# tech-srl/code2vec

Hardware: NVIDIA H100
Metric: path-contexts/sec (train step, batch 1024x200) (higher is better)
Workload: dtype tf32 operands / fp32 accumulate+storage

## Files before the change

### code2vec_b200/csrc/engine.cu

```cuda
#include <cuda_runtime.h>
#include <math.h>
#include <stdio.h>
#include <stdlib.h>
#include <string.h>

#include <string>
#include <utility>
#include <vector>

#include "../../include/c2v_b200.h"
#include "common.cuh"
#include "kernels.cuh"
#include "sgemm.cuh"
#include "umma_gemm.cuh"

using namespace c2v;

namespace {

thread_local std::string g_create_error = "";

constexpr size_t kAlign = 256;
inline size_t align_up(size_t x, size_t a = kAlign) { return (x + a - 1) / a * a; }

constexpr int kSplitDv = 18;
constexpr int kSplitDw = 48;

struct Workspace {
  size_t H, Xg, dXg, alpha, v, dv, S, loss_b, lse, loss, part, da_part, lse_part, dl;
  size_t Xg_lo, H_lo, S_lo, tgt_hi, tgt_lo, W_hi, W_lo, v_hi, v_lo;
  size_t WT, WT_lo, vT, vT_lo, tgtT, tgtT_lo;
  size_t true_logit, rscale, v_scaled, slab_flag;
  size_t st_src, st_pth, st_tgt, st_mask, st_target, st_topk_idx, st_topk_val, st_code, st_attn;
  size_t nx_src, nx_pth, nx_tgt;
  size_t sb_src, sb_pth, sb_tgt, sb_mask, sb_target;
  size_t stamp_tok, stamp_path, last_tok, last_path, lr_tab;
  size_t stamp_tgt, last_tgt;
  size_t perm, bkt_count, bkt_cursor, bkt_starts;
  size_t det_keys[2], det_vals[2], det_hist, det_offs, det_starts, det_part;
  size_t total;
  size_t ldS;
  size_t ldB;
};

bool dims_ok(const c2v_dims* d, std::string* why) {
  auto bad = [&](const char* m) { if (why) *why = m; return false; };
  if (!d) return bad("dims is NULL");
  if (d->token_vocab < 1 || d->path_vocab < 1 || d->target_vocab < 1) return bad("vocab sizes must be >= 1");
  if (d->embed_dim < 4 || d->embed_dim % 4) return bad("embed_dim must be a positive multiple of 4");
  if (d->code_dim < 4 || d->code_dim % 4 || d->code_dim > 1024) return bad("code_dim must be a multiple of 4 in [4, 1024]");
  if (d->max_contexts < 1) return bad("max_contexts must be >= 1");
  if (d->max_batch < 1) return bad("max_batch must be >= 1");
  if (d->top_k < 1 || d->top_k > 64) return bad("top_k must be in [1, 64]");
  if ((double)d->max_batch * d->max_contexts > 2.0e9) return bad("max_batch * max_contexts overflows int32");
  return true;
}

Workspace carve(const c2v_dims& d) {
  Workspace w{};
  const size_t N = (size_t)d.max_batch * d.max_contexts, D = d.code_dim, B = d.max_batch, X = 3 * (size_t)d.embed_dim;
  w.ldS = align_up((size_t)d.target_vocab, 64);
  w.ldB = align_up(B, 4);
  size_t off = 0;
  auto take = [&](size_t bytes) { size_t o = off; off = align_up(off + bytes); return o; };
  w.H = take(N * D * 4);
  w.Xg = take(N * X * 4);
  w.dXg = take(N * X * 4);
  w.alpha = take(N * 4);
  w.v = take(B * D * 4);
  w.dv = take(B * D * 4);
  w.S = take(B * w.ldS * 4);
  w.loss_b = take(B * 4);
  w.lse = take(B * 4);
  w.true_logit = take(B * 4);
  w.rscale = take(B * 4);
  w.v_scaled = take(B * D * 4);
  w.slab_flag = take(64);
  w.loss = take(64);
  size_t part = (size_t)kSplitDv * B * D;
  if ((size_t)kSplitDw * X * D > part) part = (size_t)kSplitDw * X * D;
  w.part = take(part * 4);
  w.da_part = take(B * D * 4);
  w.lse_part = take(B * (size_t)umma::lse_slots(d.target_vocab) * 8);
  w.dl = take(B * (size_t)(kMaxSampled + 1) * 4);
  w.st_src = take(N * 4);
  w.st_pth = take(N * 4);
  w.st_tgt = take(N * 4);
  w.st_mask = take(N * 4);
  w.nx_src = take(N * 4);
  w.nx_pth = take(N * 4);
  w.nx_tgt = take(N * 4);
  w.st_target = take(B * 4);
  w.sb_src = take(N * 4);
  w.sb_pth = take(N * 4);
  w.sb_tgt = take(N * 4);
  w.sb_mask = take(N * 4);
  w.sb_target = take(B * 4);
  w.st_topk_idx = take(B * (size_t)d.top_k * 4);
  w.st_topk_val = take(B * (size_t)d.top_k * 4);
  w.st_code = take(B * D * 4);
  w.st_attn = take(N * 4);
  w.stamp_tok = take((size_t)d.token_vocab * 4);
  w.stamp_path = take((size_t)d.path_vocab * 4);
  w.last_tok = take((size_t)d.token_vocab * 4);
  w.last_path = take((size_t)d.path_vocab * 4);
  w.lr_tab = take((size_t)kLrRing * 4);
  w.perm = take(3 * N * 4);
  w.bkt_count = take((size_t)kMaxBuckets * 4);
  w.bkt_cursor = take((size_t)kMaxBuckets * 4);
  w.bkt_starts = take((size_t)(kMaxBuckets + 1) * 4);
  w.stamp_tgt = take((size_t)d.target_vocab * 4);
  w.last_tgt = take((size_t)d.target_vocab * 4);
  w.Xg_lo = take(N * X * 4);
  w.H_lo = take(N * D * 4);
  w.S_lo = take(B * w.ldS * 4);
  w.tgt_hi = take((size_t)d.target_vocab * D * 4);
  w.tgt_lo = take((size_t)d.target_vocab * D * 4);
  w.W_hi = take(X * D * 4);
  w.W_lo = take(X * D * 4);
  w.v_hi = take(B * D * 4);
  w.v_lo = take(B * D * 4);
  w.WT = take(X * D * 4);
  w.WT_lo = take(X * D * 4);
  w.vT = take(D * w.ldB * 4);
  w.vT_lo = take(D * w.ldB * 4);
  w.tgtT = take(D * w.ldS * 4);
  w.tgtT_lo = take(D * w.ldS * 4);
  const size_t M = 3 * N, tiles = (M + kDetSortTile - 1) / kDetSortTile;
  for (int i = 0; i < 2; ++i) { w.det_keys[i] = take(M * 4); w.det_vals[i] = take(M * 4); }
  w.det_hist = take(kDetRadix * tiles * 4);
  w.det_offs = take(kDetRadix * tiles * 4);
  w.det_starts = take((kDetRadix * tiles + 1) * 4);
  w.det_part = take(2 * ((M + kDetChunk - 1) / kDetChunk) * (size_t)d.embed_dim * 4);
  w.total = off;
  return w;
}

}

enum Phase { PH_CTX_FWD = 0, PH_ATTN_FWD, PH_LOGITS, PH_XENT, PH_DV, PH_DY, PH_ATTN_BWD, PH_DW, PH_DX_SCATTER,
             PH_ADAM, PH_TOPK, PH_SAMPLED, PH_GATHER, PH_DX_GEMM, PH_ADAM_CATCHUP, PH_SPLIT, PH_ADAM_SWEEP, PH_PEER_SORT, PH_INBOX_APPLY,
             PH_COUNT };
const char* const kPhaseNames[PH_COUNT] = {"ctx_fwd", "attn_fwd", "logits", "xent", "dv", "dY", "attn_bwd", "dW",
                                           "dx_scatter", "adam", "topk", "sampled_softmax", "gather", "dx_gemm",
                                           "adam_catchup", "split", "adam_sweep", "peer_sort", "inbox_apply"};
struct PhaseLog {
  std::vector<std::pair<cudaEvent_t, cudaEvent_t>> pending;
  std::vector<std::pair<cudaEvent_t, cudaEvent_t>> free_list;
  double total_ms = 0.0;
  int64_t count = 0;
};

enum HeadSchedule {
  HEAD_SIMT,
  HEAD_TWO_PASS,
  HEAD_LOADERS,
  HEAD_RECOMPUTE,
  HEAD_EXP_SLAB,
};

struct SlabDesc {
  const float* row_scale = nullptr;
  bool loaders = false;
  umma::SoftmaxGradArgs sg{};
};

struct PendingDy {
  const float* v = nullptr;
  int B = 0;
  SlabDesc slab;
};

struct c2v_engine {
  PhaseLog phase[PH_COUNT];
  int profile = 0;
  c2v_dims dims;
  int device;
  Workspace ws;
  char* wbase;
  size_t wbytes;
  c2v_tensors theta, grad, am, av;
  ShardedTable th_tok{}, th_path{}, gr_tok{}, gr_path{};
  int table_world = 1;
  float grad_scale = 1.f;
  int lazy = 0;
  int adam_rows_occ = 4;
  int sweep_period = 32;
  int64_t full_flush_t = 0;
  int rest_shortcut = 1;
  bool tgt_lazy = false;
  bool tgt_t_valid = false;
  bool lazy_grads_pending = false;
  int64_t adam_t_done = 0;
  int32_t mark_epoch = 0;
  float hp_lr = 0.f, hp_b1 = 0.f, hp_b2 = 0.f, hp_eps = 0.f;
  bool hp_set = false;
  bool has_theta, has_grad, has_adam;
  bool emb_grads_clean;
  int math_mode;
  const int32_t* sorted_src = nullptr;
  int sorted_rows = 0;
  InboxSet inbox{};
  int ordered_exchange = 0;
  bool exchange_pushed = false;
  int sort_peer = 1;
  bool bkt_zeroed = false;
  int recompute = 0;
  int exp_slab = 1;
  bool slab_flag_zeroed = false;
  HeadSchedule split_fwd = HEAD_SIMT;
  int gather_occ[2] = {0, 0};
  int adam_epi_prefetch = 0;
  int fuse_sg = 0;
  int fuse_gather = 0;
  int cta_pair = 2;
  int num_sms;
  cudaEvent_t ev_tgt_ready = nullptr;
  int dy_late = 1;
  PendingDy pending_dy;
  cudaStream_t side = nullptr;
  cudaEvent_t ev_fork = nullptr, ev_join = nullptr;
  cudaStream_t copy = nullptr;
  cudaEvent_t ev_h2d[2] = {nullptr, nullptr}, ev_used[2] = {nullptr, nullptr};
  bool used_valid[2] = {false, false};
  uint64_t async_n = 0;
  cudaStream_t side2 = nullptr;
  cudaEvent_t ev_fork2 = nullptr, ev_join2 = nullptr;
  bool dy_in_flight = false;
  bool tgt_armed = false;
  float tgt_lr = 0.f, tgt_b1 = 0.f, tgt_b2 = 0.f, tgt_eps = 0.f;
  int64_t tgt_t = 0;
  int64_t armed_t = 0;
  const int32_t* hint_src = nullptr;
  const int32_t* hint_pth = nullptr;
  const int32_t* hint_tgt = nullptr;
  int hint_B = 0;
  int64_t early_t = 0;
  int64_t early_count = 0;
  int fuse_tgt = 0;
  int64_t tgt_fused_t = 0;
  int deterministic;
  int64_t launches;
  std::string err;
};

namespace {

int fail(c2v_engine* e, int code, const std::string& msg) {
  if (e) e->err = msg; else g_create_error = msg;
  return code;
}

struct PhaseTimer {
  c2v_engine* e; int ph; cudaStream_t st; cudaEvent_t stop = nullptr;
  PhaseTimer(c2v_engine* e_, int ph_, cudaStream_t st_) : e(e_), ph(ph_), st(st_) {
    if (!e->profile) return;
    PhaseLog& L = e->phase[ph];
    std::pair<cudaEvent_t, cudaEvent_t> ev;
    if (!L.free_list.empty()) { ev = L.free_list.back(); L.free_list.pop_back(); }
    else { cudaEventCreate(&ev.first); cudaEventCreate(&ev.second); }
    cudaEventRecord(ev.first, st);
    stop = ev.second;
    L.pending.push_back(ev);
  }
  ~PhaseTimer() { if (stop) cudaEventRecord(stop, st); }
};

#define C2V_CUDA(e, expr)                                                                         \
  do {                                                                                            \
    cudaError_t _c = (expr);                                                                      \
    if (_c != cudaSuccess)                                                                        \
      return fail((e), C2V_ERR_CUDA, std::string(#expr) + ": " + cudaGetErrorString(_c));         \
  } while (0)

#define C2V_LAUNCH(e, ...)                                                                        \
  do {                                                                                            \
    __VA_ARGS__;                                                                                  \
    cudaError_t _c = cudaGetLastError();                                                          \
    if (_c != cudaSuccess)                                                                        \
      return fail((e), C2V_ERR_CUDA, std::string("kernel launch failed: ") + cudaGetErrorString(_c)); \
    (e)->launches++;                                                                              \
  } while (0)

#define C2V_ADAM_ROWS(e, MODE, stream, ...)                                                                    \
  do {                                                                                                         \
    if ((e)->adam_rows_occ == 5)                                                                               \
      C2V_LAUNCH(e, (adam_rows_kernel<MODE, 5><<<(e)->num_sms * 5, 256, 0, stream>>>(__VA_ARGS__)));           \
    else                                                                                                       \
      C2V_LAUNCH(e, (adam_rows_kernel<MODE, 4><<<(e)->num_sms * 4, 256, 0, stream>>>(__VA_ARGS__)));           \
  } while (0)

inline int rest_ok(const c2v_engine* e) {
  return (e->rest_shortcut && e->hp_b1 > 0.f && e->hp_b1 <= 0.95f && e->hp_b2 >= 0.99f && e->hp_b2 < 1.f && e->hp_eps > 0.f) ? 1 : 0;
}
// ... 44 lines not shown
int check_batch(c2v_engine* e, int32_t B) {
  if (!e) return C2V_ERR_INVALID;
  if (B < 1 || B > e->dims.max_batch) return fail(e, C2V_ERR_INVALID, "batch size out of range [1, max_batch]");
  if (!e->wbase) return fail(e, C2V_ERR_STATE, "workspace not bound (c2v_bind_workspace)");
  if (!e->has_theta) return fail(e, C2V_ERR_STATE, "parameters not bound (c2v_bind_params)");
  return C2V_OK;
}

int launch_attn_fwd(c2v_engine* e, cudaStream_t st, const float* H, const float* mask, int B, float* alpha, float* v) {
  const int C = e->dims.max_contexts, D = e->dims.code_dim;
  const size_t smem = ((size_t)((C + 3) & ~3) + 32 + kAttnWarps + (size_t)kAttnWarps * D) * sizeof(float);
  const float* a = e->theta.a;
  PhaseTimer pt(e, PH_ATTN_FWD, st);
#define C2V_AF(NV)                                                                                        \
  do {                                                                                                    \
    if (smem > 48 * 1024)                                                                                 \
      C2V_CUDA(e, cudaFuncSetAttribute(attn_fwd_kernel<NV>, cudaFuncAttributeMaxDynamicSharedMemorySize, (int)smem)); \
    C2V_LAUNCH(e, (attn_fwd_kernel<NV><<<B, kAttnThreads, smem, st>>>(H, a, mask, C, D, alpha, v)));      \
  } while (0)
  switch ((D + 127) / 128) {
    case 1: C2V_AF(1); break;
    case 2: C2V_AF(2); break;
    case 3: C2V_AF(3); break;
    case 4: C2V_AF(4); break;
    case 5: case 6: C2V_AF(6); break;
    default: C2V_AF(8); break;
  }
#undef C2V_AF
  return C2V_OK;
}

int launch_attn_bwd(c2v_engine* e, cudaStream_t st, float* H, const float* alpha, const float* dv, const float* v, int B,
                    float* da_part, float* H_lo) {
  const int C = e->dims.max_contexts, D = e->dims.code_dim;
  const size_t smem = (size_t)kAttnWarps * D * sizeof(float);
  const float* a = e->theta.a;
  PhaseTimer pt(e, PH_ATTN_BWD, st);
#define C2V_AB(NV)                                                                                        \
  do {                                                                                                    \
    if (H_lo) {                                                                                           \
      if (smem > 48 * 1024)                                                                               \
        C2V_CUDA(e, cudaFuncSetAttribute(attn_bwd_kernel<NV, true>, cudaFuncAttributeMaxDynamicSharedMemorySize, (int)smem)); \
      C2V_LAUNCH(e, (attn_bwd_kernel<NV, true><<<B, kAttnThreads, smem, st>>>(H, alpha, dv, v, a, C, D, da_part, H_lo))); \
    } else {                                                                                              \
      if (smem > 48 * 1024)                                                                               \
        C2V_CUDA(e, cudaFuncSetAttribute(attn_bwd_kernel<NV, false>, cudaFuncAttributeMaxDynamicSharedMemorySize, (int)smem)); \
      C2V_LAUNCH(e, (attn_bwd_kernel<NV, false><<<B, kAttnThreads, smem, st>>>(H, alpha, dv, v, a, C, D, da_part, nullptr))); \
    }                                                                                                     \
  } while (0)
  switch ((D + 127) / 128) {
    case 1: C2V_AB(1); break;
    case 2: C2V_AB(2); break;
    case 3: C2V_AB(3); break;
    case 4: C2V_AB(4); break;
    case 5: case 6: C2V_AB(6); break;
    default: C2V_AB(8); break;
  }
#undef C2V_AB
  return C2V_OK;
}

int launch_colsum(c2v_engine* e, cudaStream_t st, const float* in, size_t stride, int R, int n, float* out,
                  const float* row_scale = nullptr, int row_len = 0) {
  if (R <= 64 && n % 4 == 0 && stride % 4 == 0 && (!row_scale || row_len % 4 == 0)) {
    size_t blocks = ((size_t)n / 4 + 255) / 256;
    if (blocks > (size_t)e->num_sms * 16) blocks = (size_t)e->num_sms * 16;
    C2V_LAUNCH(e, (slice_sum_kernel<<<(unsigned)blocks, 256, 0, st>>>(in, stride, R, (size_t)n / 4, out, row_scale, row_scale ? row_len / 4 : 1)));
    return C2V_OK;
  }
  C2V_LAUNCH(e, (colsum_kernel<<<(n + 31) / 32, dim3(32, 32), 0, st>>>(in, stride, R, n, out)));
  if (row_scale) C2V_LAUNCH(e, (scale_rows_kernel<<<(unsigned)(((size_t)n + 255) / 256), 256, 0, st>>>(out, row_scale, out, row_len, (size_t)n)));
  return C2V_OK;
}

ContextSource make_source(c2v_engine* e, const int32_t* src, const int32_t* pth, const int32_t* tgt, int B) {
  ContextSource cs{};
  cs.src = src; cs.pth = pth; cs.tgt = tgt;
  cs.tok = e->th_tok; cs.path = e->th_path;
  cs.d = e->dims.embed_dim;
  cs.rows = B * e->dims.max_contexts;
  return cs;
}

int prepare_rows(c2v_engine* e, cudaStream_t st, const ContextSource& cs) {
  if (!e->lazy) return C2V_OK;
  PhaseTimer pt(e, PH_ADAM_CATCHUP, st);
  const c2v_dims& d = e->dims;
  int32_t* stamp_tok = wsp<int32_t>(e, e->ws.stamp_tok);
  int32_t* stamp_path = wsp<int32_t>(e, e->ws.stamp_path);
  e->mark_epoch++;
  C2V_LAUNCH(e, (mark_rows_kernel<<<(cs.rows + 255) / 256, 256, 0, st>>>(cs.src, cs.pth, cs.tgt, cs.rows, stamp_tok, stamp_path,
                                                                        e->mark_epoch)));
  if (e->adam_t_done > 0) {
    const float* lr_tab = wsp<float>(e, e->ws.lr_tab);
    C2V_ADAM_ROWS(e, ADAM_ROWS_CATCHUP, st,
                  e->theta.tok, e->grad.tok, e->am.tok, e->av.tok, d.token_vocab, d.embed_dim, stamp_tok, e->mark_epoch,
                      wsp<int32_t>(e, e->ws.last_tok), (int32_t)e->adam_t_done, lr_tab, e->hp_b1, e->hp_b2, e->hp_eps, rest_ok(e));
    C2V_ADAM_ROWS(e, ADAM_ROWS_CATCHUP, st,
                  e->theta.path, e->grad.path, e->am.path, e->av.path, d.path_vocab, d.embed_dim, stamp_path, e->mark_epoch,
                      wsp<int32_t>(e, e->ws.last_path), (int32_t)e->adam_t_done, lr_tab, e->hp_b1, e->hp_b2, e->hp_eps, rest_ok(e));
  }
  return C2V_OK;
}

int launch_sweep(c2v_engine* e, cudaStream_t st, float* p, float* g, float* m, float* v, int rows, int dim, int32_t* last, int64_t t) {
  if (rows <= 0) return C2V_OK;
  int blocks = (rows + 7) / 8;
  if (blocks > e->num_sms * 4) blocks = e->num_sms * 4;
  C2V_LAUNCH(e, (adam_sweep_kernel<4><<<blocks, 256, 0, st>>>(p, g, m, v, rows, dim, last, (int32_t)t, wsp<float>(e, e->ws.lr_tab), e->hp_b1,
                                                             e->hp_b2, e->hp_eps, rest_ok(e))));
  return C2V_OK;
}

int flush_rows(c2v_engine* e, cudaStream_t st) {
  if (!e->lazy || e->adam_t_done == 0) return C2V_OK;
  const c2v_dims& d = e->dims;
  const float* lr_tab = wsp<float>(e, e->ws.lr_tab);
  { int rcw = launch_sweep(e, st, e->theta.tok, e->grad.tok, e->am.tok, e->av.tok, d.token_vocab, d.embed_dim, wsp<int32_t>(e, e->ws.last_tok), e->adam_t_done);
    if (rcw) return rcw; }
  { int rcw = launch_sweep(e, st, e->theta.path, e->grad.path, e->am.path, e->av.path, d.path_vocab, d.embed_dim, wsp<int32_t>(e, e->ws.last_path), e->adam_t_done);
    if (rcw) return rcw; }
  if (e->tgt_lazy)
    { int rcw = launch_sweep(e, st, e->theta.tgt, e->grad.tgt, e->am.tgt, e->av.tgt, d.target_vocab, d.code_dim, wsp<int32_t>(e, e->ws.last_tgt), e->adam_t_done);
    if (rcw) return rcw; }
  e->full_flush_t = e->adam_t_done;
  return C2V_OK;
}

int end_target_lazy(c2v_engine* e, cudaStream_t st) {
  if (!e->tgt_lazy) return C2V_OK;
  if (e->adam_t_done > 0) {
    const c2v_dims& d = e->dims;
    { int rcw = launch_sweep(e, st, e->theta.tgt, e->grad.tgt, e->am.tgt, e->av.tgt, d.target_vocab, d.code_dim, wsp<int32_t>(e, e->ws.last_tgt), e->adam_t_done);
    if (rcw) return rcw; }
  }
  e->tgt_lazy = false;
  return C2V_OK;
}

int sweep_rows(c2v_engine* e, cudaStream_t st, int64_t t) {
  const int R = e->sweep_period;
  if (!e->lazy || R <= 0) return C2V_OK;
  if (R == 1) return flush_rows(e, st);
  PhaseTimer pt(e, PH_ADAM_SWEEP, st);
  const c2v_dims& d = e->dims;
  const float* lr_tab = wsp<float>(e, e->ws.lr_tab);
  const int64_t ph = t % R;
  auto slice = [&](float* p, float* g, float* m, float* v, int rows, int dim, int32_t* last) -> int {
    const int64_t lo = (int64_t)rows * ph / R, hi = (int64_t)rows * (ph + 1) / R;
    if (hi <= lo) return C2V_OK;
    const size_t o = (size_t)lo * dim;
    return launch_sweep(e, st, p + o, g + o, m + o, v + o, (int)(hi - lo), dim, last + lo, t);
  };
  int rc;
  if ((rc = slice(e->theta.tok, e->grad.tok, e->am.tok, e->av.tok, d.token_vocab, d.embed_dim, wsp<int32_t>(e, e->ws.last_tok)))) return rc;
  if ((rc = slice(e->theta.path, e->grad.path, e->am.path, e->av.path, d.path_vocab, d.embed_dim, wsp<int32_t>(e, e->ws.last_path)))) return rc;
  if (e->tgt_lazy &&
      (rc = slice(e->theta.tgt, e->grad.tgt, e->am.tgt, e->av.tgt, d.target_vocab, d.code_dim, wsp<int32_t>(e, e->ws.last_tgt)))) return rc;
  if (ph == R - 1) e->full_flush_t = t - R + 1;
  return C2V_OK;
}

int early_catchup(c2v_engine* e, cudaStream_t side) {
  const int32_t *hs = e->hint_src, *hp = e->hint_pth, *ht = e->hint_tgt;
  const int hB = e->hint_B;
  e->hint_src = e->hint_pth = e->hint_tgt = nullptr;
  e->hint_B = 0;
  if (!hs || !e->lazy || e->table_world > 1) return C2V_OK;
  const int64_t t = e->armed_t;
  if (t != e->adam_t_done + 1) return C2V_OK;
  if (!e->hp_set || e->tgt_lr != e->hp_lr || e->tgt_b1 != e->hp_b1 || e->tgt_b2 != e->hp_b2 || e->tgt_eps != e->hp_eps)
    return C2V_OK;
  const c2v_dims& d = e->dims;
  const double lr_t = (double)e->tgt_lr * sqrt(1.0 - pow((double)e->tgt_b2, (double)t)) / (1.0 - pow((double)e->tgt_b1, (double)t));
  float* lr_tab = wsp<float>(e, e->ws.lr_tab);
  int32_t* stamp_tok = wsp<int32_t>(e, e->ws.stamp_tok);
  int32_t* stamp_path = wsp<int32_t>(e, e->ws.stamp_path);
  PhaseTimer pt(e, PH_ADAM_CATCHUP, side);
  C2V_LAUNCH(e, (set_float_kernel<<<1, 1, 0, side>>>(lr_tab + (t & kLrRingMask), (float)lr_t)));
  e->mark_epoch++;
  const int rows = hB * d.max_contexts;
  C2V_LAUNCH(e, (mark_rows_kernel<<<(rows + 255) / 256, 256, 0, side>>>(hs, hp, ht, rows, stamp_tok, stamp_path, e->mark_epoch)));
  C2V_ADAM_ROWS(e, ADAM_ROWS_CATCHUP, side,
                  e->theta.tok, e->grad.tok, e->am.tok, e->av.tok, d.token_vocab, d.embed_dim, stamp_tok, e->mark_epoch,
                    wsp<int32_t>(e, e->ws.last_tok), (int32_t)t, lr_tab, e->hp_b1, e->hp_b2, e->hp_eps, rest_ok(e));
  C2V_ADAM_ROWS(e, ADAM_ROWS_CATCHUP, side,
                  e->theta.path, e->grad.path, e->am.path, e->av.path, d.path_vocab, d.embed_dim, stamp_path, e->mark_epoch,
                    wsp<int32_t>(e, e->ws.last_path), (int32_t)t, lr_tab, e->hp_b1, e->hp_b2, e->hp_eps, rest_ok(e));
  e->early_t = t;
  e->early_count++;
  return C2V_OK;
}

int split_small(c2v_engine* e, cudaStream_t st, const float* x, size_t n, size_t off_hi, size_t off_lo) {
  PhaseTimer pt(e, PH_SPLIT, st);
  const size_t n4 = n / 4;
  size_t blocks = (n4 + 255) / 256;
  if (blocks > (size_t)e->num_sms * 16) blocks = (size_t)e->num_sms * 16;
  if (blocks < 1) blocks = 1;
  C2V_LAUNCH(e, (split_tf32_kernel<<<(unsigned)blocks, 256, 0, st>>>(x, wsp<float>(e, off_hi), wsp<float>(e, off_lo), n4)));
  return C2V_OK;
}

int transpose_operand(c2v_engine* e, cudaStream_t st, const float* x, int rows, int cols, size_t ldT, size_t off_t, bool split,
                      size_t off_lo = 0, float* hi = nullptr, float* lo = nullptr) {
  const dim3 grid((unsigned)((rows + 31) / 32), (unsigned)((cols + 31) / 32));
  if (split)
    C2V_LAUNCH(e, (transpose_kernel<true><<<grid, 256, 0, st>>>(x, rows, cols, wsp<float>(e, off_t), wsp<float>(e, off_lo), ldT, hi, lo)));
  else
    C2V_LAUNCH(e, (transpose_kernel<false><<<grid, 256, 0, st>>>(x, rows, cols, wsp<float>(e, off_t), nullptr, ldT, nullptr, nullptr)));
  return C2V_OK;
}

int transpose_table(c2v_engine* e, cudaStream_t st) {
  const int Y = e->dims.target_vocab, D = e->dims.code_dim;
  int rc;
  if (is_3x(e)) {
    PhaseTimer pt(e, PH_SPLIT, st);
    rc = transpose_operand(e, st, e->theta.tgt, Y, D, e->ws.ldS, e->ws.tgtT, true, e->ws.tgtT_lo);
  } else {
    PhaseTimer pt(e, PH_DV, st);
    rc = transpose_operand(e, st, e->theta.tgt, Y, D, e->ws.ldS, e->ws.tgtT, false);
  }
  if (rc) return rc;
  e->tgt_t_valid = true;
  return C2V_OK;
}

bool plan_buckets(c2v_engine* e, BucketPlan* bp, bool force = false) {
  if (e->table_world <= 1) return false;
  const c2v_dims& d = e->dims;
  const double table_bytes = ((double)d.token_vocab + d.path_vocab) * d.embed_dim * 4.0;
  if (!force && (e->sort_peer == 0 || (e->sort_peer == 1 && table_bytes < 2.0e9))) return false;
  const int W = e->table_world;
  int rows_per_page = (int)((2u << 20) / ((size_t)d.embed_dim * 4));
  int ps = 0;
  while ((2 << ps) <= rows_per_page) ++ps;
  bp->shift = e->th_tok.shift; bp->mask = e->th_tok.mask; bp->page_shift = ps;
  const int rows_tok = (d.token_vocab + W - 1) / W, rows_path = (d.path_vocab + W - 1) / W;
  bp->pages_tok = (rows_tok >> ps) + 1;
  bp->pages_path = (rows_path >> ps) + 1;
  bp->n_buckets = W * (bp->pages_tok + bp->pages_path);
  return bp->n_buckets <= kMaxBuckets;
}
int sort_entries(c2v_engine* e, cudaStream_t st, const ContextSource& cs, const BucketPlan& bp) {
  PhaseTimer pt(e, PH_PEER_SORT, st);
  int32_t* counts = wsp<int32_t>(e, e->ws.bkt_count);
  int32_t* cursor = wsp<int32_t>(e, e->ws.bkt_cursor);
  if (!e->bkt_zeroed) {
    C2V_CUDA(e, cudaMemsetAsync(counts, 0, (size_t)kMaxBuckets * 4, st));
    e->bkt_zeroed = true;
  }
  const int total = 3 * cs.rows;
  int blocks = (total + 255) / 256;
  if (blocks > e->num_sms * 8) blocks = e->num_sms * 8;
  C2V_LAUNCH(e, (bucket_count_kernel<<<blocks, 256, (size_t)bp.n_buckets * 4, st>>>(cs, bp, counts)));
  C2V_LAUNCH(e, (bucket_scan_kernel<<<1, 1024, 0, st>>>(counts, cursor, wsp<int32_t>(e, e->ws.bkt_starts), bp.n_buckets)));
  C2V_LAUNCH(e, (bucket_fill_kernel<<<blocks, 256, 0, st>>>(cs, bp, cursor, wsp<int32_t>(e, e->ws.perm))));
  return C2V_OK;
}

template <class KeyFn>
int det_sort(c2v_engine* e, cudaStream_t st, const KeyFn& key, int count, uint32_t nkeys, int* cur_out) {
  int bits = 1;
  while (bits < 32 && (1ull << bits) <= nkeys) ++bits;
  uint32_t* keys[2] = {wsp<uint32_t>(e, e->ws.det_keys[0]), wsp<uint32_t>(e, e->ws.det_keys[1])};
  int32_t* vals[2] = {wsp<int32_t>(e, e->ws.det_vals[0]), wsp<int32_t>(e, e->ws.det_vals[1])};
  int32_t* hist = wsp<int32_t>(e, e->ws.det_hist);
  int32_t* offs = wsp<int32_t>(e, e->ws.det_offs);
  int blocks = (count + 255) / 256;
  if (blocks > e->num_sms * 8) blocks = e->num_sms * 8;
// ... 1676 lines not shown
```

### code2vec_b200/csrc/kernels.cuh

```cuda
#pragma once
#include <float.h>
#include <limits.h>
#include "common.cuh"

namespace c2v {

constexpr int kAttnThreads = 128;
constexpr int kAttnWarps = kAttnThreads / 32;

__device__ __forceinline__ float block_sum(float v, float* red) {
  const int lane = threadIdx.x & 31, warp = threadIdx.x >> 5, nw = (blockDim.x + 31) >> 5;
  v = warp_sum(v);
  __syncthreads();
  if (lane == 0) red[warp] = v;
  __syncthreads();
  float r = (threadIdx.x < nw) ? red[threadIdx.x] : 0.f;
  if (warp == 0) {
    r = warp_sum(r);
    if (lane == 0) red[0] = r;
  }
  __syncthreads();
  r = red[0];
  __syncthreads();
  return r;
// ... 1077 lines not shown
}

__global__ void inbox_counts_kernel(const __grid_constant__ InboxSet inbox, const __grid_constant__ BucketPlan bp,
                                    const int32_t* __restrict__ starts) {
  const int o = threadIdx.x;
  if (o > bp.mask) return;
  const int W = bp.mask + 1, t0 = o * bp.pages_tok, p0 = W * bp.pages_tok + o * bp.pages_path;
  InboxView v = inbox_of(inbox, o);
  v.cnt[2 * inbox.rank] = starts[t0 + bp.pages_tok] - starts[t0];
  v.cnt[2 * inbox.rank + 1] = starts[p0 + bp.pages_path] - starts[p0];
}

__global__ void __launch_bounds__(256)
scatter_inbox_kernel(const __grid_constant__ ContextSource cs, const __grid_constant__ Dropout dp, const float* __restrict__ mask,
                     const int32_t* __restrict__ perm, const int32_t* __restrict__ starts, const __grid_constant__ BucketPlan bp,
                     const float* __restrict__ dXg, const __grid_constant__ InboxSet inbox, float grad_scale) {
  const int w = blockIdx.x * 8 + (threadIdx.x >> 5), lane = threadIdx.x & 31;
  if (w >= 3 * cs.rows) return;
  const int e = perm[w];
  const int n = e / 3, seg = e - 3 * n;
  const int idx = seg == 0 ? cs.src[n] : (seg == 1 ? cs.pth[n] : cs.tgt[n]);
  const int o = idx & bp.mask, W = bp.mask + 1;
  const int t0 = o * bp.pages_tok, p0 = W * bp.pages_tok + o * bp.pages_path;
  const int k = (seg == 1) ? (starts[t0 + bp.pages_tok] - starts[t0]) + (w - starts[p0]) : (w - starts[t0]);
  InboxView v = inbox_of(inbox, o);
  const size_t slot = (size_t)inbox.rank * inbox.cap + k;
  const bool live = mask[n] != 0.f;
  if (lane == 0) v.ids[slot] = live ? (idx >> bp.shift) : -1;
  if (!live) return;
  const float* src = dXg + (size_t)n * (3 * cs.d) + (size_t)seg * cs.d;
  float* dst = v.val + slot * cs.d;
  for (int j = lane * 4; j < cs.d; j += 128) {
    float4 g = *reinterpret_cast<const float4*>(src + j);
    const float4 m = dropout_mult4(dp, n, (seg * cs.d + j) >> 2);
    g.x *= m.x * grad_scale; g.y *= m.y * grad_scale; g.z *= m.z * grad_scale; g.w *= m.w * grad_scale;
    *reinterpret_cast<float4*>(dst + j) = g;
  }
}

__global__ void __launch_bounds__(256)
inbox_apply_kernel(const __grid_constant__ InboxSet inbox, int d, float* __restrict__ g_tok, float* __restrict__ g_path) {
  const int lane = threadIdx.x & 31;
  const int warp_global = (blockIdx.x * 256 + threadIdx.x) >> 5, total_warps = (gridDim.x * 256) >> 5;
  InboxView v = inbox_of(inbox, inbox.rank);
  for (int s = 0; s < inbox.world; ++s) {
    const int n_tok = v.cnt[2 * s], n_all = n_tok + v.cnt[2 * s + 1];
    for (int k = warp_global; k < n_all; k += total_warps) {
      const size_t slot = (size_t)s * inbox.cap + k;
      const int row = v.ids[slot];
      if (row < 0) continue;
      float* dst = (k < n_tok ? g_tok : g_path) + (size_t)row * d;
      const float* src = v.val + slot * d;
      for (int j = lane * 4; j < d; j += 128) atomicAdd(reinterpret_cast<float4*>(dst + j), *reinterpret_cast<const float4*>(src + j));
    }
  }
}

__global__ void __launch_bounds__(256)
mark_rows_kernel(const int32_t* __restrict__ src, const int32_t* __restrict__ pth, const int32_t* __restrict__ tgt, int n,
                 int32_t* __restrict__ stamp_tok, int32_t* __restrict__ stamp_path, int32_t epoch) {
  const int i = blockIdx.x * 256 + threadIdx.x;
  if (i >= n) return;
  stamp_tok[src[i]] = epoch;
  stamp_path[pth[i]] = epoch;
  stamp_tok[tgt[i]] = epoch;
}

__global__ void __launch_bounds__(256)
mark_list_kernel(const int32_t* __restrict__ idx, int n, int32_t* __restrict__ stamp, int32_t epoch) {
  const int i = blockIdx.x * 256 + threadIdx.x;
  if (i < n) stamp[idx[i]] = epoch;
}

__global__ void fill_i32_kernel(int32_t* __restrict__ p, size_t n, int32_t v) {
  for (size_t i = (size_t)blockIdx.x * blockDim.x + threadIdx.x; i < n; i += (size_t)gridDim.x * blockDim.x) p[i] = v;
}
__global__ void set_float_kernel(float* p, float v) { *p = v; }

enum { ADAM_ROWS_CATCHUP = 0, ADAM_ROWS_FLUSH = 2 };

constexpr int kLrRing = 1 << 16;
constexpr int kLrRingMask = kLrRing - 1;

__device__ __forceinline__ void replay_row(float* __restrict__ p, float* __restrict__ g, float* __restrict__ m, float* __restrict__ v,
                                           size_t row_off, int d, int32_t from, int32_t t_done, const float* __restrict__ lr_tab,
                                           float b1, float b2, float eps, float omb1, float omb2, int lane, bool rest_ok) {
  for (int j0 = 0; j0 < d; j0 += 128) {
    const int j = j0 + lane * 4;
    const bool act = j < d;
    const size_t o = row_off + (act ? j : 0);
    float4 P = make_float4(0.f, 0.f, 0.f, 0.f), M = P, V = P, G = P;
    if (act) {
      P = *reinterpret_cast<float4*>(p + o); M = *reinterpret_cast<float4*>(m + o); V = *reinterpret_cast<float4*>(v + o);
      G = *reinterpret_cast<const float4*>(g + o);
    }
    float* pp = reinterpret_cast<float*>(&P);
    float* mm = reinterpret_cast<float*>(&M);
    float* vv = reinterpret_cast<float*>(&V);
    const float* gg = reinterpret_cast<const float*>(&G);
    {
      const float lr_s = lr_tab[(from + 1) & kLrRingMask];
#pragma unroll
      for (int q = 0; q < 4; ++q) {
        mm[q] = __fadd_rn(__fmul_rn(mm[q], b1), __fmul_rn(omb1, gg[q]));
        vv[q] = __fadd_rn(__fmul_rn(vv[q], b2), __fmul_rn(omb2, __fmul_rn(gg[q], gg[q])));
        pp[q] = adam_move(pp[q], lr_s, mm[q], vv[q], eps);
      }
    }
    int32_t s = from + 2;
    for (; s <= t_done; ++s) {
      const float lr_s = lr_tab[s & kLrRingMask];
      bool moved = false;
#pragma unroll
      for (int q = 0; q < 4; ++q) {
        mm[q] = __fadd_rn(__fmul_rn(mm[q], b1), __fmul_rn(omb1, 0.f));
        vv[q] = __fadd_rn(__fmul_rn(vv[q], b2), __fmul_rn(omb2, 0.f));
        const float np = adam_move(pp[q], lr_s, mm[q], vv[q], eps);
        moved |= (__float_as_uint(np) != __float_as_uint(pp[q]));
        pp[q] = np;
      }
      if (rest_ok && !__any_sync(0xffffffffu, moved)) { ++s; break; }
    }
    for (; s <= t_done; ++s) {
#pragma unroll
      for (int q = 0; q < 4; ++q) {
        mm[q] = __fadd_rn(__fmul_rn(mm[q], b1), __fmul_rn(omb1, 0.f));
        vv[q] = __fadd_rn(__fmul_rn(vv[q], b2), __fmul_rn(omb2, 0.f));
      }
    }
    if (act) {
      *reinterpret_cast<float4*>(p + o) = P;
      *reinterpret_cast<float4*>(m + o) = M;
      *reinterpret_cast<float4*>(v + o) = V;
      if ((__float_as_uint(G.x) | __float_as_uint(G.y) | __float_as_uint(G.z) | __float_as_uint(G.w)) != 0u)
        *reinterpret_cast<float4*>(g + o) = make_float4(0.f, 0.f, 0.f, 0.f);
    }
  }
}

template <int MODE, int OCC>
__global__ void __launch_bounds__(256, OCC)
adam_rows_kernel(float* __restrict__ p, float* __restrict__ g, float* __restrict__ m, float* __restrict__ v, int rows, int d,
                 const int32_t* __restrict__ stamp, int32_t epoch, int32_t* __restrict__ last, int32_t t_done,
                 const float* __restrict__ lr_tab, float b1, float b2, float eps, int rest_ok) {
  const int lane = threadIdx.x & 31;
  const int warp_global = (blockIdx.x * 256 + threadIdx.x) >> 5;
  const int total_warps = (gridDim.x * 256) >> 5;
  const float omb1 = __fsub_rn(1.f, b1), omb2 = __fsub_rn(1.f, b2);
  for (int base = warp_global * 32; base < rows; base += total_warps * 32) {
    const int r = base + lane;
    int32_t from_l = 0;
    bool hit = false;
    if (r < rows) {
      hit = (MODE == ADAM_ROWS_FLUSH) || (stamp[r] == epoch);
      if (hit) {
        from_l = last[r];
        if (from_l >= t_done) hit = false;
      }
    }
    unsigned todo = __ballot_sync(0xffffffffu, hit);
    auto prefetch_row = [&](int row) {
      const size_t o = (size_t)row * d + lane * 4;
      if (lane * 4 < d) {
        asm volatile("prefetch.global.L2 [%0];" ::"l"(p + o));
        asm volatile("prefetch.global.L2 [%0];" ::"l"(m + o));
        asm volatile("prefetch.global.L2 [%0];" ::"l"(v + o));
        asm volatile("prefetch.global.L2 [%0];" ::"l"(g + o));
      }
    };
    if (todo) prefetch_row(base + __ffs(todo) - 1);
    while (todo) {
      const int b = __ffs(todo) - 1;
      todo &= todo - 1;
      if (todo) prefetch_row(base + __ffs(todo) - 1);
      const int32_t from = __shfl_sync(0xffffffffu, from_l, b);
      replay_row(p, g, m, v, (size_t)(base + b) * d, d, from, t_done, lr_tab, b1, b2, eps, omb1, omb2, lane, rest_ok != 0);
    }
    if (hit) last[r] = t_done;
  }
}

template <int OCC>
__global__ void __launch_bounds__(256, OCC)
adam_sweep_kernel(float* __restrict__ p, float* __restrict__ g, float* __restrict__ m, float* __restrict__ v, int rows, int d,
                  int32_t* __restrict__ last, int32_t t_done, const float* __restrict__ lr_tab, float b1, float b2, float eps,
                  int rest_ok) {
  const int lane = threadIdx.x & 31;
  const int warp_global = (blockIdx.x * 256 + threadIdx.x) >> 5;
  const int total_warps = (gridDim.x * 256) >> 5;
  const float omb1 = __fsub_rn(1.f, b1), omb2 = __fsub_rn(1.f, b2);
  for (int row = warp_global; row < rows; row += total_warps) {
    const int32_t from = last[row];
    if (from >= t_done) continue;
    replay_row(p, g, m, v, (size_t)row * d, d, from, t_done, lr_tab, b1, b2, eps, omb1, omb2, lane, rest_ok != 0);
    __syncwarp();
    if (lane == 0) last[row] = t_done;
  }
}

constexpr int kDetChunk = 32;
constexpr int kDetSortThreads = 256;
constexpr int kDetSortTile = 4096;
constexpr int kDetRadix = 256;

struct DetStepKeys {
  const int32_t* src;
  const int32_t* pth;
  const int32_t* tgt;
  const float* mask;
  int T;
  uint32_t nkeys;
  __device__ __forceinline__ uint32_t operator()(int e) const {
    const int n = e / 3, seg = e - 3 * n;
    if (mask[n] == 0.f) return nkeys;
    return seg == 1 ? (uint32_t)(T + pth[n]) : (uint32_t)(seg == 0 ? src[n] : tgt[n]);
  }
};
struct DetListKeys {
  const int32_t* rows;
  int base;
  __device__ __forceinline__ uint32_t operator()(int e) const { return (uint32_t)(base + rows[e]); }
};

template <class KeyFn>
__global__ void __launch_bounds__(256)
det_keys_kernel(const __grid_constant__ KeyFn key, int count, uint32_t* __restrict__ keys, int32_t* __restrict__ vals) {
  for (int e = blockIdx.x * 256 + threadIdx.x; e < count; e += gridDim.x * 256) {
    keys[e] = key(e);
    vals[e] = e;
  }
}

__global__ void __launch_bounds__(kDetSortThreads)
det_hist_kernel(const uint32_t* __restrict__ keys, int count, int shift, int32_t* __restrict__ hist) {
  __shared__ int32_t h[kDetRadix];
  h[threadIdx.x] = 0;
  __syncthreads();
  const int lo = blockIdx.x * kDetSortTile, hi = min(count, lo + kDetSortTile);
  for (int i = lo + threadIdx.x; i < hi; i += kDetSortThreads) atomicAdd(&h[(keys[i] >> shift) & (kDetRadix - 1)], 1);
  __syncthreads();
  hist[threadIdx.x * gridDim.x + blockIdx.x] = h[threadIdx.x];
}

__global__ void __launch_bounds__(kDetSortThreads)
det_scatter_kernel(const uint32_t* __restrict__ keys, const int32_t* __restrict__ vals, int count, int shift,
                   const int32_t* __restrict__ offs, uint32_t* __restrict__ okeys, int32_t* __restrict__ ovals) {
  constexpr int W = kDetSortThreads / 32;
  __shared__ int32_t wc[W][kDetRadix];
  __shared__ int32_t run[kDetRadix];
  __shared__ int32_t goff[kDetRadix];
  const int tid = threadIdx.x, lane = tid & 31, warp = tid >> 5;
  run[tid] = 0;
  goff[tid] = offs[tid * gridDim.x + blockIdx.x];
  const int lo = blockIdx.x * kDetSortTile, hi = min(count, lo + kDetSortTile);
  for (int base = lo; base < hi; base += kDetSortThreads) {
#pragma unroll
    for (int w = 0; w < W; ++w) wc[w][tid] = 0;
    __syncthreads();
    const int i = base + tid;
    const bool valid = i < hi;
    const uint32_t k = valid ? keys[i] : 0u;
    const int q = valid ? (int)((k >> shift) & (kDetRadix - 1)) : kDetRadix + lane;
    const unsigned peers = __match_any_sync(0xffffffffu, q);
    const int rank = __popc(peers & ((1u << lane) - 1u));
// ... 326 lines not shown
```

Before: 32.04 million.

## Compact touched rows into a list and replay Adam catch-up with cp.async ring

Replaces the two per-table lazy-Adam catch-up launches with a compaction kernel that collects stale touched rows from both token and path tables into one list, plus a list-driven kernel. The new kernel prefetches p/m/v/g slices through a per-warp cp.async shared-memory ring while replaying the deferred Adam steps. The goal is to drop the warp-per-vocab-row scan, balance work across both tables in one grid, and hide global-memory latency. In exchange it adds a global atomic counter, a memset, an extra launch and dynamic shared memory that may reduce occupancy.

```diff
diff --git a/code2vec_b200/csrc/engine.cu b/code2vec_b200/csrc/engine.cu
--- a/code2vec_b200/csrc/engine.cu
+++ b/code2vec_b200/csrc/engine.cu
@@ -36,6 +36,7 @@
   size_t sb_src, sb_pth, sb_tgt, sb_mask, sb_target;
   size_t stamp_tok, stamp_path, last_tok, last_path, lr_tab;
   size_t stamp_tgt, last_tgt;
+  size_t catchup_list, catchup_count;
   size_t perm, bkt_count, bkt_cursor, bkt_starts;
   size_t det_keys[2], det_vals[2], det_hist, det_offs, det_starts, det_part;
   size_t total;
@@ -105,6 +106,8 @@
   w.last_tok = take((size_t)d.token_vocab * 4);
   w.last_path = take((size_t)d.path_vocab * 4);
   w.lr_tab = take((size_t)kLrRing * 4);
+  w.catchup_list = take(std::min((size_t)d.token_vocab + d.path_vocab, 3 * N) * sizeof(uint2));
+  w.catchup_count = take(64);
   w.perm = take(3 * N * 4);
   w.bkt_count = take((size_t)kMaxBuckets * 4);
   w.bkt_cursor = take((size_t)kMaxBuckets * 4);
@@ -210,6 +213,7 @@
   bool slab_flag_zeroed = false;
   HeadSchedule split_fwd = HEAD_SIMT;
   int gather_occ[2] = {0, 0};
+  int catchup_occ = 0;
   int adam_epi_prefetch = 0;
   int fuse_sg = 0;
   int fuse_gather = 0;
@@ -420,24 +424,39 @@
   return cs;
 }
 
+int launch_catchup(c2v_engine* e, cudaStream_t st, int32_t t_done) {
+  const c2v_dims& d = e->dims;
+  CatchupTables tb{};
+  tb.p[0] = e->theta.tok; tb.g[0] = e->grad.tok; tb.m[0] = e->am.tok; tb.v[0] = e->av.tok;
+  tb.p[1] = e->theta.path; tb.g[1] = e->grad.path; tb.m[1] = e->am.path; tb.v[1] = e->av.path;
+  tb.stamp[0] = wsp<int32_t>(e, e->ws.stamp_tok); tb.stamp[1] = wsp<int32_t>(e, e->ws.stamp_path);
+  tb.last[0] = wsp<int32_t>(e, e->ws.last_tok); tb.last[1] = wsp<int32_t>(e, e->ws.last_path);
+  tb.rows[0] = d.token_vocab; tb.rows[1] = d.path_vocab;
+  uint2* list = wsp<uint2>(e, e->ws.catchup_list);
+  int* count = wsp<int>(e, e->ws.catchup_count);
+  if (e->catchup_occ == 0) {
+    C2V_CUDA(e, cudaFuncSetAttribute(adam_list_kernel, cudaFuncAttributeMaxDynamicSharedMemorySize, kCatchupSmem));
+    int n = 0;
+    C2V_CUDA(e, cudaOccupancyMaxActiveBlocksPerMultiprocessor(&n, adam_list_kernel, 256, kCatchupSmem));
+    e->catchup_occ = n > 0 ? n : 1;
+  }
+  C2V_CUDA(e, cudaMemsetAsync(count, 0, sizeof(int), st));
+  const unsigned rows = (unsigned)d.token_vocab + (unsigned)d.path_vocab;
+  C2V_LAUNCH(e, (catchup_list_kernel<<<(rows + 255) / 256, 256, 0, st>>>(tb, e->mark_epoch, t_done, list, count)));
+  C2V_LAUNCH(e, (adam_list_kernel<<<e->num_sms * e->catchup_occ, 256, kCatchupSmem, st>>>(
+      tb, d.embed_dim, list, count, t_done, wsp<float>(e, e->ws.lr_tab), e->hp_b1, e->hp_b2, e->hp_eps, rest_ok(e))));
+  return C2V_OK;
+}
+
 int prepare_rows(c2v_engine* e, cudaStream_t st, const ContextSource& cs) {
   if (!e->lazy) return C2V_OK;
   PhaseTimer pt(e, PH_ADAM_CATCHUP, st);
-  const c2v_dims& d = e->dims;
   int32_t* stamp_tok = wsp<int32_t>(e, e->ws.stamp_tok);
   int32_t* stamp_path = wsp<int32_t>(e, e->ws.stamp_path);
   e->mark_epoch++;
   C2V_LAUNCH(e, (mark_rows_kernel<<<(cs.rows + 255) / 256, 256, 0, st>>>(cs.src, cs.pth, cs.tgt, cs.rows, stamp_tok, stamp_path,
                                                                         e->mark_epoch)));
-  if (e->adam_t_done > 0) {
-    const float* lr_tab = wsp<float>(e, e->ws.lr_tab);
-    C2V_ADAM_ROWS(e, ADAM_ROWS_CATCHUP, st,
-                  e->theta.tok, e->grad.tok, e->am.tok, e->av.tok, d.token_vocab, d.embed_dim, stamp_tok, e->mark_epoch,
-                      wsp<int32_t>(e, e->ws.last_tok), (int32_t)e->adam_t_done, lr_tab, e->hp_b1, e->hp_b2, e->hp_eps, rest_ok(e));
-    C2V_ADAM_ROWS(e, ADAM_ROWS_CATCHUP, st,
-                  e->theta.path, e->grad.path, e->am.path, e->av.path, d.path_vocab, d.embed_dim, stamp_path, e->mark_epoch,
-                      wsp<int32_t>(e, e->ws.last_path), (int32_t)e->adam_t_done, lr_tab, e->hp_b1, e->hp_b2, e->hp_eps, rest_ok(e));
-  }
+  if (e->adam_t_done > 0) return launch_catchup(e, st, (int32_t)e->adam_t_done);
   return C2V_OK;
 }
 
@@ -519,12 +538,7 @@
   e->mark_epoch++;
   const int rows = hB * d.max_contexts;
   C2V_LAUNCH(e, (mark_rows_kernel<<<(rows + 255) / 256, 256, 0, side>>>(hs, hp, ht, rows, stamp_tok, stamp_path, e->mark_epoch)));
-  C2V_ADAM_ROWS(e, ADAM_ROWS_CATCHUP, side,
-                  e->theta.tok, e->grad.tok, e->am.tok, e->av.tok, d.token_vocab, d.embed_dim, stamp_tok, e->mark_epoch,
-                    wsp<int32_t>(e, e->ws.last_tok), (int32_t)t, lr_tab, e->hp_b1, e->hp_b2, e->hp_eps, rest_ok(e));
-  C2V_ADAM_ROWS(e, ADAM_ROWS_CATCHUP, side,
-                  e->theta.path, e->grad.path, e->am.path, e->av.path, d.path_vocab, d.embed_dim, stamp_path, e->mark_epoch,
-                    wsp<int32_t>(e, e->ws.last_path), (int32_t)t, lr_tab, e->hp_b1, e->hp_b2, e->hp_eps, rest_ok(e));
+  { int rc = launch_catchup(e, side, (int32_t)t); if (rc) return rc; }
   e->early_t = t;
   e->early_count++;
   return C2V_OK;
diff --git a/code2vec_b200/csrc/kernels.cuh b/code2vec_b200/csrc/kernels.cuh
--- a/code2vec_b200/csrc/kernels.cuh
+++ b/code2vec_b200/csrc/kernels.cuh
@@ -1183,6 +1183,45 @@
 constexpr int kLrRing = 1 << 16;
 constexpr int kLrRingMask = kLrRing - 1;
 
+__device__ __forceinline__ void replay_slice(float4& P, float4& M, float4& V, const float4& G, int32_t from, int32_t t_done,
+                                             const float* __restrict__ lr_tab, float b1, float b2, float eps, float omb1,
+                                             float omb2, bool rest_ok) {
+  float* pp = reinterpret_cast<float*>(&P);
+  float* mm = reinterpret_cast<float*>(&M);
+  float* vv = reinterpret_cast<float*>(&V);
+  const float* gg = reinterpret_cast<const float*>(&G);
+  {
+    const float lr_s = lr_tab[(from + 1) & kLrRingMask];
+#pragma unroll
+    for (int q = 0; q < 4; ++q) {
+      mm[q] = __fadd_rn(__fmul_rn(mm[q], b1), __fmul_rn(omb1, gg[q]));
+      vv[q] = __fadd_rn(__fmul_rn(vv[q], b2), __fmul_rn(omb2, __fmul_rn(gg[q], gg[q])));
+      pp[q] = adam_move(pp[q], lr_s, mm[q], vv[q], eps);
+    }
+  }
+  int32_t s = from + 2;
+  for (; s <= t_done; ++s) {
+    const float lr_s = lr_tab[s & kLrRingMask];
+    bool moved = false;
+#pragma unroll
+    for (int q = 0; q < 4; ++q) {
+      mm[q] = __fadd_rn(__fmul_rn(mm[q], b1), __fmul_rn(omb1, 0.f));
+      vv[q] = __fadd_rn(__fmul_rn(vv[q], b2), __fmul_rn(omb2, 0.f));
+      const float np = adam_move(pp[q], lr_s, mm[q], vv[q], eps);
+      moved |= (__float_as_uint(np) != __float_as_uint(pp[q]));
+      pp[q] = np;
+    }
+    if (rest_ok && !__any_sync(0xffffffffu, moved)) { ++s; break; }
+  }
+  for (; s <= t_done; ++s) {
+#pragma unroll
+    for (int q = 0; q < 4; ++q) {
+      mm[q] = __fadd_rn(__fmul_rn(mm[q], b1), __fmul_rn(omb1, 0.f));
+      vv[q] = __fadd_rn(__fmul_rn(vv[q], b2), __fmul_rn(omb2, 0.f));
+    }
+  }
+}
+
 __device__ __forceinline__ void replay_row(float* __restrict__ p, float* __restrict__ g, float* __restrict__ m, float* __restrict__ v,
                                            size_t row_off, int d, int32_t from, int32_t t_done, const float* __restrict__ lr_tab,
                                            float b1, float b2, float eps, float omb1, float omb2, int lane, bool rest_ok) {
@@ -1195,40 +1234,7 @@
       P = *reinterpret_cast<float4*>(p + o); M = *reinterpret_cast<float4*>(m + o); V = *reinterpret_cast<float4*>(v + o);
       G = *reinterpret_cast<const float4*>(g + o);
     }
-    float* pp = reinterpret_cast<float*>(&P);
-    float* mm = reinterpret_cast<float*>(&M);
-    float* vv = reinterpret_cast<float*>(&V);
-    const float* gg = reinterpret_cast<const float*>(&G);
-    {
-      const float lr_s = lr_tab[(from + 1) & kLrRingMask];
-#pragma unroll
-      for (int q = 0; q < 4; ++q) {
-        mm[q] = __fadd_rn(__fmul_rn(mm[q], b1), __fmul_rn(omb1, gg[q]));
-        vv[q] = __fadd_rn(__fmul_rn(vv[q], b2), __fmul_rn(omb2, __fmul_rn(gg[q], gg[q])));
-        pp[q] = adam_move(pp[q], lr_s, mm[q], vv[q], eps);
-      }
-    }
-    int32_t s = from + 2;
-    for (; s <= t_done; ++s) {
-      const float lr_s = lr_tab[s & kLrRingMask];
-      bool moved = false;
-#pragma unroll
-      for (int q = 0; q < 4; ++q) {
-        mm[q] = __fadd_rn(__fmul_rn(mm[q], b1), __fmul_rn(omb1, 0.f));
-        vv[q] = __fadd_rn(__fmul_rn(vv[q], b2), __fmul_rn(omb2, 0.f));
-        const float np = adam_move(pp[q], lr_s, mm[q], vv[q], eps);
-        moved |= (__float_as_uint(np) != __float_as_uint(pp[q]));
-        pp[q] = np;
-      }
-      if (rest_ok && !__any_sync(0xffffffffu, moved)) { ++s; break; }
-    }
-    for (; s <= t_done; ++s) {
-#pragma unroll
-      for (int q = 0; q < 4; ++q) {
-        mm[q] = __fadd_rn(__fmul_rn(mm[q], b1), __fmul_rn(omb1, 0.f));
-        vv[q] = __fadd_rn(__fmul_rn(vv[q], b2), __fmul_rn(omb2, 0.f));
-      }
-    }
+    replay_slice(P, M, V, G, from, t_done, lr_tab, b1, b2, eps, omb1, omb2, rest_ok);
     if (act) {
       *reinterpret_cast<float4*>(p + o) = P;
       *reinterpret_cast<float4*>(m + o) = M;
@@ -1281,6 +1287,108 @@
   }
 }
 
+struct CatchupTables {
+  float* p[2];
+  float* g[2];
+  float* m[2];
+  float* v[2];
+  const int32_t* stamp[2];
+  int32_t* last[2];
+  int rows[2];
+};
+constexpr int kCatchupRing = 3;
+constexpr int kCatchupSmem = 8 * kCatchupRing * 4 * 128 * 4;
+
+__global__ void __launch_bounds__(256)
+catchup_list_kernel(const __grid_constant__ CatchupTables tb, int32_t epoch, int32_t t_done, uint2* __restrict__ list,
+                    int* __restrict__ count) {
+  __shared__ int warp_off[8], block_off;
+  const int i = blockIdx.x * 256 + threadIdx.x, lane = threadIdx.x & 31, w = threadIdx.x >> 5;
+  const int tab = i < tb.rows[0] ? 0 : 1;
+  const int r = tab ? i - tb.rows[0] : i;
+  bool hit = false;
+  int32_t from = 0;
+  if (r < tb.rows[tab] && tb.stamp[tab][r] == epoch) {
+    from = tb.last[tab][r];
+    hit = from < t_done;
+  }
+  const unsigned bal = __ballot_sync(0xffffffffu, hit);
+  if (lane == 0) warp_off[w] = __popc(bal);
+  __syncthreads();
+  if (threadIdx.x == 0) {
+    int n = 0;
+    for (int k = 0; k < 8; ++k) { const int c = warp_off[k]; warp_off[k] = n; n += c; }
+    block_off = n ? atomicAdd(count, n) : 0;
+  }
+  __syncthreads();
+  if (hit) {
+    list[block_off + warp_off[w] + __popc(bal & ((1u << lane) - 1u))] = make_uint2(((uint32_t)r << 1) | (uint32_t)tab, (uint32_t)from);
+    tb.last[tab][r] = t_done;
+  }
+}
+
+__device__ __forceinline__ void cp_async16(void* smem, const void* gmem) {
+  asm volatile("cp.async.cg.shared.global [%0], [%1], 16;" ::"r"((uint32_t)__cvta_generic_to_shared(smem)), "l"(gmem) : "memory");
+}
+
+__global__ void __launch_bounds__(256)
+adam_list_kernel(const __grid_constant__ CatchupTables tb, int d, const uint2* __restrict__ list, const int* __restrict__ count,
+                 int32_t t_done, const float* __restrict__ lr_tab, float b1, float b2, float eps, int rest_ok) {
+  extern __shared__ float4 ring[];
+  const int lane = threadIdx.x & 31;
+  float4* mine = ring + (threadIdx.x >> 5) * (kCatchupRing * 4 * 32) + lane;
+  const long long stride = (gridDim.x * 256) >> 5;
+  const long long first = (blockIdx.x * 256 + threadIdx.x) >> 5;
+  const int slices = (d + 127) / 128;
+  const long long items = (long long)*count * slices;
+  const float omb1 = __fsub_rn(1.f, b1), omb2 = __fsub_rn(1.f, b2);
+  auto locate = [&](long long it, int& tab, size_t& o, int32_t& from) -> bool {
+    const uint2 en = list[it / slices];
+    const int j = (int)(it % slices) * 128 + lane * 4;
+    tab = (int)(en.x & 1u);
+    from = (int32_t)en.y;
+    o = (size_t)(en.x >> 1) * d + (j < d ? j : 0);
+    return j < d;
+  };
+  auto issue = [&](long long it, int slot) {
+    if (it < items) {
+      int tab; size_t o; int32_t from;
+      if (locate(it, tab, o, from)) {
+        float4* s = mine + slot * 128;
+        cp_async16(s, tb.p[tab] + o);
+        cp_async16(s + 32, tb.m[tab] + o);
+        cp_async16(s + 64, tb.v[tab] + o);
+        cp_async16(s + 96, tb.g[tab] + o);
+      }
+    }
+    asm volatile("cp.async.commit_group;" ::: "memory");
+  };
+#pragma unroll
+  for (int k = 0; k < kCatchupRing - 1; ++k) issue(first + k * stride, k);
+  int slot = 0;
+  for (long long it = first; it < items; it += stride) {
+    issue(it + (kCatchupRing - 1) * stride, slot == 0 ? kCatchupRing - 1 : slot - 1);
+    asm volatile("cp.async.wait_group %0;" ::"n"(kCatchupRing - 1) : "memory");
+    int tab; size_t o; int32_t from;
+    const bool act = locate(it, tab, o, from);
+    float4 P = make_float4(0.f, 0.f, 0.f, 0.f), M = P, V = P, G = P;
+    if (act) {
+      const float4* s = mine + slot * 128;
+      P = s[0]; M = s[32]; V = s[64]; G = s[96];
+    }
+    replay_slice(P, M, V, G, from, t_done, lr_tab, b1, b2, eps, omb1, omb2, rest_ok != 0);
+    if (act) {
+      *reinterpret_cast<float4*>(tb.p[tab] + o) = P;
+      *reinterpret_cast<float4*>(tb.m[tab] + o) = M;
+      *reinterpret_cast<float4*>(tb.v[tab] + o) = V;
+      if ((__float_as_uint(G.x) | __float_as_uint(G.y) | __float_as_uint(G.z) | __float_as_uint(G.w)) != 0u)
+        *reinterpret_cast<float4*>(tb.g[tab] + o) = make_float4(0.f, 0.f, 0.f, 0.f);
+    }
+    slot = slot == kCatchupRing - 1 ? 0 : slot + 1;
+  }
+  asm volatile("cp.async.wait_all;" ::: "memory");
+}
+
 template <int OCC>
 __global__ void __launch_bounds__(256, OCC)
 adam_sweep_kernel(float* __restrict__ p, float* __restrict__ g, float* __restrict__ m, float* __restrict__ v, int rows, int d,
```

After: 32.33 million, median of 6. Within noise of the previous version (+0.9%).
